# eloialonso/diamond

Measured on AMD Instinct MI355X. Metric: imagined frames/sec (64x64, 3 denoise steps, batch 256), higher is better.
Workload: dtype f32 via split-f16 MFMA (world-model convs (3x3 stride 1 / 2, 1x1): fp32 operands split into 2 x fp16 pieces, 3 x v_mfma_f32_*_f16 per product, fp32 accumulate (fp32-class, 22-bit operands); attention core, linears: exact fp32 v_mfma_f32_16x16x4_f32; actor-critic encoder forward, dgrad and weight-gra

## Files before the change

### diamond_amd/csrc/dmd_conv_f16ws.hip

```cpp
#include <type_traits>

#include "dmd_common.h"

typedef _Float16 h8 __attribute__((ext_vector_type(8)));
typedef _Float16 h4 __attribute__((ext_vector_type(4)));
typedef _Float16 h2 __attribute__((ext_vector_type(2)));
typedef float f32x16 __attribute__((ext_vector_type(16)));
typedef unsigned int u32x4 __attribute__((ext_vector_type(4)));

#ifdef DMD_LAB
#ifndef WS_ABL
#define WS_ABL 0
#endif
#else
#undef WS_ABL
#define WS_ABL 0
#endif
#if defined(DMD_LAB) && defined(WS_WRITEOUT_PRIO)
#define WS_PRIO_COMPUTE() __builtin_amdgcn_s_setprio(3)
#define WS_PRIO_WRITEOUT() __builtin_amdgcn_s_setprio(WS_WRITEOUT_PRIO)
#else
#define WS_PRIO_COMPUTE() do {} while (0)
#define WS_PRIO_WRITEOUT() do {} while (0)
#endif

template <bool B8_, int NCB_, int TAPS_ = 9>
struct WsGeom {
  static constexpr int NPT = 256;
  static constexpr bool B8 = B8_;
  static constexpr int NCB = NCB_;
  static constexpr int TAPS = TAPS_;
  static constexpr int COUT = 32 * NCB_;
  static constexpr int NPH = 4 / NCB_;
  static constexpr int SUB = B8_ ? 2 * NPH : NPH / 2;
  static constexpr int TS = B8_ ? 8 : 16;
  static constexpr int PW = TS + 2;
  static constexpr int PPS = PW * PW;
  static constexpr int NPP = SUB * PPS;
  static constexpr int ITEMS = (NPP * 4 + NPT - 1) / NPT;
  static constexpr int W_UNITS = TAPS_ * 2 * 2 * COUT;
  static constexpr int WU = (W_UNITS + 255) / 256;
  static constexpr int PATCH_BYTES = NPP * 64;
  static constexpr int W_BYTES = W_UNITS * 16;
  static constexpr int W_BASE = 2 * PATCH_BYTES;
  static constexpr int BUF_BYTES = PATCH_BYTES + W_BYTES;
  static constexpr int CIN_MAX = NCB_ == 2 ? 128 : 64;
  static constexpr int TAB_SLOTS = 4;
  static constexpr int TAB_FLOATS = TAB_SLOTS * SUB * CIN_MAX;
  static constexpr bool CD_TABLES = !(B8_ && NCB_ == 1);
  static constexpr int SMEM_BYTES = 2 * BUF_BYTES + (CD_TABLES ? 4 : 2) * TAB_FLOATS * 4 + COUT * 4;
  static constexpr bool DOUBLE_STAGE = NCB_ == 2;
  static constexpr bool ASM_LOADS = DOUBLE_STAGE;
  static constexpr int HALVES = TAPS_ * 2;
  static constexpr bool PL_REGS = !(B8_ && NCB_ == 1);
  static constexpr int blk_off(int blk) { return (B8_ ? (blk >> 1) * PPS + (blk & 1) * 4 * PW : blk * 2 * PW) * 64; }
  static constexpr bool PROJ = false;
  static constexpr int PROJ_KS = 1;
};

struct WsGeomProj : WsGeom<false, 2, 9> {
  static constexpr bool PROJ = true;
  static constexpr int PROJ_KS = 8;
  static constexpr int PROJ_BYTES = PROJ_KS * 2 * 2 * COUT * 16;
  static constexpr bool PL_REGS = false;
  static constexpr int SMEM_BYTES = WsGeom<false, 2, 9>::SMEM_BYTES + PROJ_BYTES;
};

struct WsTile {
  int n, y0, x0;
  bool valid;
};

template <class G>
__device__ __forceinline__ WsTile ws_subtile(const dmd_conv_params& p, int tile, int s) {
  const int tx = p.W / G::TS, per_img = tx * (p.H / G::TS);
  const int gs = tile * G::SUB + s;
  WsTile t;
  t.valid = gs < p.N * per_img;
  const int g2 = t.valid ? gs : 0;
  t.n = g2 / per_img;
  const int r = g2 - t.n * per_img;
  const int ty = r / tx;
  t.y0 = ty * G::TS;
  t.x0 = (r - ty * tx) * G::TS;
  return t;
}

__device__ __forceinline__ float ws_silu(float t) {
  return t * __builtin_amdgcn_rcpf(1.0f + __builtin_amdgcn_exp2f(-1.4426950408889634f * t));
}

template <int I, int N, class F>
__device__ __forceinline__ void ws_for(F&& f) {
  if constexpr (I < N) {
    f(std::integral_constant<int, I>{});
    ws_for<I + 1, N>(f);
  }
}

#ifndef WS_SYNCTHREADS
#define WS_SYNCTHREADS 0
#endif
__device__ __forceinline__ void ws_barrier() {
#if WS_SYNCTHREADS
  __syncthreads();
#else
  asm volatile("s_waitcnt lgkmcnt(0)\n\ts_barrier" ::: "memory");
#endif
}

#if defined(DMD_LAB) && defined(WS_TRACE)
#define WS_TRACE_WG (gridDim.x > 37 ? 37 : 0)
#define WS_TRACE_N 4096
__device__ unsigned long long ws_trace_buf[3][WS_TRACE_N];
__device__ int ws_trace_cnt[3];
#define WS_TRACE_DECL int ws_ti = 0
#define WS_STAMP(role_, tag_, step_)                                                                                  \
  do {                                                                                                                 \
    if (blockIdx.x == WS_TRACE_WG && (threadIdx.x & 255) == 0 && ws_ti < WS_TRACE_N) {                                  \
      ws_trace_buf[role_][ws_ti] = (__builtin_readcyclecounter() << 16) | ((unsigned long long)(tag_) << 12) | ((step_) & 0xfff); \
      ws_trace_cnt[role_] = ++ws_ti;                                                                                   \
    }                                                                                                                  \
  } while (0)
extern "C" int dmd_ws_trace_dump(unsigned long long* host, int* counts) {
  hipDeviceSynchronize();
  hipMemcpyFromSymbol(host, HIP_SYMBOL(ws_trace_buf), sizeof(unsigned long long) * 3 * WS_TRACE_N);
  hipMemcpyFromSymbol(counts, HIP_SYMBOL(ws_trace_cnt), sizeof(int) * 3);
  int zero[3] = {0, 0, 0};
  hipMemcpyToSymbol(HIP_SYMBOL(ws_trace_cnt), zero, sizeof(zero));
  return WS_TRACE_N;
}
#else
#define WS_TRACE_DECL
#define WS_STAMP(role_, tag_, step_) do {} while (0)
#endif

#ifndef WS_HOST_HELPERS
__device__ __forceinline__ void ws_aload(f32x4& dst, const f32x4* src) {
  asm volatile("global_load_dwordx4 %0, %1, off" : "=&v"(dst) : "v"(src) : "memory");
}
template <bool FIRST>
// ... 25 lines not shown
  const unsigned long long v = (unsigned long long)p;
  const unsigned lo = __builtin_amdgcn_readfirstlane((unsigned)v), hi = __builtin_amdgcn_readfirstlane((unsigned)(v >> 32));
  return (const char*)(((unsigned long long)hi << 32) | lo);
}
template <int CTRL, int ROW_MASK>
__device__ __forceinline__ double ws_dpp_add(double x) {
  const unsigned long long u = __builtin_bit_cast(unsigned long long, x);
  const unsigned lo = (unsigned)__builtin_amdgcn_update_dpp(0, (int)(unsigned)u, CTRL, ROW_MASK, 0xf, false);
  const unsigned hi = (unsigned)__builtin_amdgcn_update_dpp(0, (int)(unsigned)(u >> 32), CTRL, ROW_MASK, 0xf, false);
  return x + __builtin_bit_cast(double, (unsigned long long)lo | ((unsigned long long)hi << 32));
}
__device__ __forceinline__ double ws_wave_sum_lane63(double x) {
  x = ws_dpp_add<0xB1, 0xf>(x);
  x = ws_dpp_add<0x4E, 0xf>(x);
  x = ws_dpp_add<0x141, 0xf>(x);
  x = ws_dpp_add<0x140, 0xf>(x);
  x = ws_dpp_add<0x142, 0xa>(x);
  x = ws_dpp_add<0x143, 0xc>(x);
  return x;
}

#ifndef WS_HOST_HELPERS
template <int N, int M>
__device__ __forceinline__ void ws_await_set(f32x4 (&st)[M]) {
  static_assert(N >= 0 && N < 64, "vmcnt is a 6-bit field");
  static_assert(M == 6 || M == 7, "register sets of the double-staged geometries");
  if constexpr (M == 6)
    asm volatile("s_waitcnt vmcnt(%6) ; await %0 %1 %2 %3 %4 %5"
                 : "+v"(st[0]), "+v"(st[1]), "+v"(st[2]), "+v"(st[3]), "+v"(st[4]), "+v"(st[5]) : "n"(N) : "memory");
  else
    asm volatile("s_waitcnt vmcnt(%7) ; await %0 %1 %2 %3 %4 %5 %6"
                 : "+v"(st[0]), "+v"(st[1]), "+v"(st[2]), "+v"(st[3]), "+v"(st[4]), "+v"(st[5]), "+v"(st[6]) : "n"(N) : "memory");
}

template <int N, int M>
__device__ __forceinline__ void ws_use_all(f32x4 (&st)[M]) {
  static_assert(N <= M, "register set");
#pragma unroll
  for (int it = 0; it < N; ++it) asm volatile("; drained %0" : : "v"(st[it]));
}
#endif

struct WsA {
  h8 h, l;
};
struct WsB {
  h8 h0, h1, l0, l1;
};

struct WsAddr {
  int ph[3], pl[3];
  int w;
};

template <class G>
__device__ __forceinline__ void ws_addr_move(WsAddr& ad, int dpar) {
  const int dp = dpar * G::PATCH_BYTES, dw = dpar * G::W_BYTES;
#pragma unroll
  for (int dx = 0; dx < 3; ++dx) {
    ad.ph[dx] += dp;
    if (G::PL_REGS) ad.pl[dx] += dp;
  }
  ad.w += dw;
}

template <class G, int TAP>
struct WsWin {
  static constexpr int win = G::TAPS == 9 ? TAP : 4;
  static constexpr int dy = win / 3, dx = win % 3;
  static constexpr int off = (dy * G::PW + dx) * 64;
};

template <class G, int TAP, int BLK, bool LOW>
__device__ __forceinline__ h8 ws_read_b(const unsigned char* lds, const WsAddr& ad) {
  using Wn = WsWin<G, TAP>;
  return *(const h8*)(lds + (LOW ? (G::PL_REGS ? ad.pl[Wn::dx] : (ad.ph[Wn::dx] ^ 32)) : ad.ph[Wn::dx]) + (Wn::off + G::blk_off(BLK)));
}
template <class G, int TAP, bool LOW>
__device__ __forceinline__ h8 ws_read_a(const unsigned char* lds, const WsAddr& ad) {
  return *(const h8*)(lds + ad.w + (TAP * 2 + (LOW ? 1 : 0)) * 2 * G::COUT * 16);
}

template <class G, int P0, int NEXT, int NT, int NP0>
__device__ __forceinline__ void ws_halftap(f32x16 (&acc)[4], const WsA& a, const WsB& b, const unsigned char* lds, const WsAddr& ad,
                                           WsA& an, WsB& bn) {
#if WS_ABL & 16
  return;
#endif
  constexpr int P1 = P0 + 1, NP1 = NP0 + 1;
  acc[P0] = __builtin_amdgcn_mfma_f32_32x32x16_f16(a.h, b.h0, acc[P0], 0, 0, 0);
  if constexpr (NEXT == 3) an.h = ws_read_a<G, NT, false>(lds, ad);
  if constexpr (NEXT == 1 || NEXT == 2) bn.h0 = ws_read_b<G, NT, NP0, false>(lds, ad);
  __builtin_amdgcn_sched_barrier(0);
  acc[P1] = __builtin_amdgcn_mfma_f32_32x32x16_f16(a.h, b.h1, acc[P1], 0, 0, 0);
  if constexpr (NEXT == 3) bn.h0 = ws_read_b<G, NT, NP0, false>(lds, ad);
  if constexpr (NEXT == 1 || NEXT == 2) bn.h1 = ws_read_b<G, NT, NP1, false>(lds, ad);
  __builtin_amdgcn_sched_barrier(0);
  acc[P0] = __builtin_amdgcn_mfma_f32_32x32x16_f16(a.h, b.l0, acc[P0], 0, 0, 0);
  if constexpr (NEXT == 3) bn.h1 = ws_read_b<G, NT, NP1, false>(lds, ad);
  if constexpr (NEXT == 1 || NEXT == 2) bn.l0 = ws_read_b<G, NT, NP0, true>(lds, ad);
  __builtin_amdgcn_sched_barrier(0);
  acc[P1] = __builtin_amdgcn_mfma_f32_32x32x16_f16(a.h, b.l1, acc[P1], 0, 0, 0);
  if constexpr (NEXT == 3) bn.l0 = ws_read_b<G, NT, NP0, true>(lds, ad);
  if constexpr (NEXT == 1 || NEXT == 2) bn.l1 = ws_read_b<G, NT, NP1, true>(lds, ad);
  __builtin_amdgcn_sched_barrier(0);
  acc[P0] = __builtin_amdgcn_mfma_f32_32x32x16_f16(a.l, b.h0, acc[P0], 0, 0, 0);
  if constexpr (NEXT == 3) bn.l1 = ws_read_b<G, NT, NP1, true>(lds, ad);
  if constexpr (NEXT == 2) an.h = ws_read_a<G, NT + 1, false>(lds, ad);
  __builtin_amdgcn_sched_barrier(0);
  acc[P1] = __builtin_amdgcn_mfma_f32_32x32x16_f16(a.l, b.h1, acc[P1], 0, 0, 0);
  if constexpr (NEXT == 3) an.l = ws_read_a<G, NT, true>(lds, ad);
  if constexpr (NEXT == 2) an.l = ws_read_a<G, NT + 1, true>(lds, ad);
  __builtin_amdgcn_sched_barrier(0);
}

template <class G>
__device__ __forceinline__ void ws_chunk_body(f32x16 (&acc)[4], WsA& a, WsB& b, const unsigned char* lds, const WsAddr& ad) {
  WsA an = a;
  WsB bn = b;
  ws_for<0, G::HALVES - 1>([&](auto uc) {
    constexpr int U = decltype(uc)::value;
    constexpr int T = U / 2, H = U % 2;
    constexpr int NU = U + 1, NT = NU / 2, NH = NU % 2;
    constexpr int NEXT = (H == 0 && T + 1 < G::TAPS) ? 2 : 1;
    ws_halftap<G, 2 * H, NEXT, NT, 2 * NH>(acc, a, b, lds, ad, an, bn);
    b = bn;
    if (H == 1) a = an;
  });
}

template <class G>
__global__ __launch_bounds__(768, 3) void conv_f16ws_kernel(const dmd_conv_params p, int ntiles, int tiles_per_wg) {
  DMD_DYNAMIC_LDS(unsigned char, smem_raw);
  float* tab_a = (float*)(smem_raw + 2 * G::BUF_BYTES);
  float* tab_b = tab_a + G::TAB_FLOATS;
  float* tab_c = tab_b + G::TAB_FLOATS;
  float* tab_d = tab_c + G::TAB_FLOATS;
  float* bias_lds = tab_b + (G::CD_TABLES ? 3 : 1) * G::TAB_FLOATS;
  static_assert(G::SMEM_BYTES <= 160 * 1024, "LDS budget");
  unsigned char* proj_lds = (unsigned char*)(bias_lds + G::COUT);
  if constexpr (G::PROJ) {
    const u32x4* pwg = (const u32x4*)p.proj_w_f16;
    for (int u = (int)threadIdx.x; u < G::PROJ_BYTES / 16; u += 768) ((u32x4*)proj_lds)[u] = pwg[u];
  }

  const int role = __builtin_amdgcn_readfirstlane((int)(threadIdx.x >> 8));
  const int tid = (int)(threadIdx.x & 255);
  WS_TRACE_DECL;
  const int lane = tid & 63, wave = __builtin_amdgcn_readfirstlane(tid >> 6);
  WS_STAMP(role, 13, 0);
  const int up = p.upsample;
  const int Hs = p.H >> up, Ws = p.W >> up;
  const int Hv = p.valid_h ? p.valid_h : p.H, Wv = p.valid_w ? p.valid_w : p.W;
  const int Hvs = Hv >> up, Wvs = Wv >> up;
  const int C0 = p.src[0].C;
  const int C1 = p.nsrc > 1 ? p.src[1].C : 0;
  const int nch0 = C0 >> 4;
  const int nchunks = (C0 + C1) >> 4;
  const int tile0 = blockIdx.x * tiles_per_wg;
  const int nmy = min(tiles_per_wg, ntiles - tile0);
  const int S = nmy * nchunks;
  const int rot = (blockIdx.x * 7) % nmy;
#define WS_TILE(k) (tile0 + (((k) + rot) >= nmy ? (k) + rot - nmy : (k) + rot))

  if (role == 2) {
    const int q = tid & 3;
    constexpr bool IPOS_REGS = !(G::B8 && G::NCB == 1);
    auto ipos_calc = [&](int it, int t) -> int {
      const int pp = (it * G::NPT + t) >> 2;
      const bool ok = pp < G::NPP;
      const int s = G::SUB == 1 ? 0 : (ok ? pp / G::PPS : 0);
      const int rem = pp - s * G::PPS;
      const int py = rem / G::PW, px = rem - py * G::PW;
      return ok ? ((s << 16) | (py << 8) | px) : -1;
    };
    int ipos_[IPOS_REGS ? G::ITEMS : 1];
#pragma unroll
    for (int it = 0; it < (IPOS_REGS ? G::ITEMS : 1); ++it) ipos_[it] = ipos_calc(it, tid);
    auto ipos = [&](int it) -> int {
      if (IPOS_REGS) return ipos_[IPOS_REGS ? it : 0];
      int t = tid;
      WS_OPAQUE(t);
      return ipos_calc(it, t);
    };
    auto loff_of = [&](int it) {
      int t = tid;
      if (G::SUB > 1) WS_OPAQUE(t);
      const int qq = t & 3;
      return ((it * (G::NPT / 4) + (t >> 2)) * 4 + (((qq >> 1) + ((ipos(it) & 0xff) >> 1)) & 3)) * 2 + (qq & 1);
    };
    int gk = -1;
    int tab_n[G::SUB];
#pragma unroll
    for (int s2 = 0; s2 < G::SUB; ++s2) tab_n[s2] = -1;
    int tab_slot = -1;
    WsTile ti[G::SUB];
    int goff[G::ITEMS];
    unsigned gzero = 0;
    int gtile = 0;
    auto item_source = [&](int it, bool& inb) -> int {
      const int ip = ipos(it);
      const int s = ip >> 16, py = (ip >> 8) & 0xff, px = ip & 0xff;
      const WsTile t = G::SUB == 1 ? ti[0] : ws_subtile<G>(p, gtile, s);
      const int iy = t.y0 - 1 + py, ix = t.x0 - 1 + px;
      const bool window = G::TAPS == 9 || (py >= 1 && py <= G::TS && px >= 1 && px <= G::TS);
      inb = ip >= 0 && window && t.valid && iy >= 0 && iy < Hv && ix >= 0 && ix < Wv;
      return inb ? ((t.n * Hs + (iy >> up)) * Ws + (ix >> up)) : 0;
    };

    auto setup_tile = [&](int k) {
// ... 162 lines not shown
          }
#else
#pragma unroll
          for (int el = 0; el < 4; ++el) {
            const float y = t[i][el] * u[i][el];
            u[i][el] = zero ? 0.f : y;
          }
#endif
        }
        __builtin_amdgcn_sched_barrier(0);
#endif
#pragma unroll
        for (int i = 0; i < NB; ++i) {
          const int it = I0 + i;
          const float* x = u[i];
          const unsigned h01 = __builtin_bit_cast(unsigned, (h2){(_Float16)x[0], (_Float16)x[1]});
          const unsigned h23 = __builtin_bit_cast(unsigned, (h2){(_Float16)x[2], (_Float16)x[3]});
          const unsigned l01 = ws_low_pair(x[0], x[1], h01);
          const unsigned l23 = ws_low_pair(x[2], x[3], h23);
          if ((it + 1) * G::NPT <= G::NPP * 4 || ipos(it) >= 0) {
            const int lo = loff_of(it);
            pb[lo] = (uint2){h01, h23};
            pb[lo ^ 4] = (uint2){l01, l23};
          }
        }
        __builtin_amdgcn_sched_barrier(0);
      });
      if constexpr (BATCH != G::ITEMS) reissue();
    };

    f32x4 stage0[G::ITEMS], stage1[G::DOUBLE_STAGE ? G::ITEMS : 1];
    unsigned zm0 = 0, zm1 = 0;
    int sl0 = 0, sl1 = 0;
    if constexpr (G::DOUBLE_STAGE) {
      issue_S(0, stage0, zm0, sl0);
      issue_S(1, stage1, zm1, sl1);
      WS_STAMP(2, 14, 0);
      ws_barrier();
      WS_STAMP(2, 15, 0);
      stage_S(0, stage0, zm0, sl0, 2);
      WS_STAMP(2, 12, 0);
      ws_barrier();
      for (int j = 0; j < S; j += 2) {
        WS_STAMP(2, 0, j);
        if (j + 1 < S) {
          stage_S(j + 1, stage1, zm1, sl1, j + 3);
          WS_STAMP(2, 1, j);
          WS_STAMP(2, 2, j);
        }
        ws_barrier();
        WS_STAMP(2, 3, j);
        if (j + 1 < S) {
          WS_STAMP(2, 0, j + 1);
          if (j + 2 < S) {
            stage_S(j + 2, stage0, zm0, sl0, j + 4);
            WS_STAMP(2, 1, j + 1);
            WS_STAMP(2, 2, j + 1);
          }
          ws_barrier();
          WS_STAMP(2, 3, j + 1);
        }
      }
      if constexpr (G::ASM_LOADS) {
        WS_WAIT_VM(0);
        ws_use_all<G::ITEMS>(stage0);
        ws_use_all<G::ITEMS>(stage1);
      }
    } else {
      issue_S(0, stage0, zm0, sl0);
      ws_barrier();
      stage_S(0, stage0, zm0, sl0, S > 1 ? 1 : -1);
      ws_barrier();
      for (int j = 0; j < S; ++j) {
        WS_STAMP(2, 0, j);
        if (j + 1 < S) {
          stage_S(j + 1, stage0, zm0, sl0, j + 2 < S ? j + 2 : -1);
          WS_STAMP(2, 1, j);
          WS_STAMP(2, 2, j);
        }
        ws_barrier();
        WS_STAMP(2, 3, j);
      }
    }
  } else {
    __builtin_amdgcn_s_setprio(3);
    const int cb = wave % G::NCB;
    const int ph = wave / G::NCB;
    const int n31 = lane & 31, g = lane >> 5;
    WsAddr ad;
    {
      const int col = G::B8 ? (n31 & 7) : (n31 & 15);
      const int pixbase = G::B8 ? (ph * 2 * G::PPS + (n31 >> 3) * G::PW + col)
                                : ((ph >> 1) * G::PPS + ((ph & 1) * 8 + (n31 >> 4)) * G::PW + col);
#pragma unroll
      for (int dx = 0; dx < 3; ++dx) {
        ad.ph[dx] = (pixbase * 4 + ((g + ((col + dx) >> 1)) & 3)) * 16;
        ad.pl[dx] = ad.ph[dx] ^ 32;
      }
      ad.w = G::W_BASE + (g * G::COUT + cb * 32 + n31) * 16;
    }
    int apar = 0;
    const unsigned char* lds = smem_raw;

    f32x16 acc[4];

    constexpr int NPO = G::B8 ? 2 : 1;
    int pixoff_[NPO];
    auto pixoff_of = [&](int blk) {
      const int base = pixoff_[G::B8 ? (blk >> 1) : 0];
      const int rows = G::B8 ? (blk & 1) * 4 : blk * 2;
      return base < 0 ? -1 : base + rows * p.W * (G::COUT / 4);
    };
    int dead = 0;
    constexpr int NSTAT = G::B8 ? 2 : 1;
    int stat_slot[NSTAT];
    using StatAcc = std::conditional_t<G::B8 || G::PROJ, float, double>;
    StatAcc ssum[NSTAT], ssq[NSTAT];
    int pending = 4;
    constexpr bool RES_PREFETCH = G::NCB == 2 && !G::PROJ;
    f32x4 rnext[4];
    auto res_prefetch = [&](int blk) __attribute__((always_inline)) {
      const int po = pixoff_of(blk);
#pragma unroll
      for (int qd = 0; qd < 4; ++qd)
        rnext[qd] = (p.residual && po >= 0 && !(WS_ABL & 128)) ? *(const f32x4*)(p.residual + (size_t)po * 4 + 8 * qd) : (f32x4){0.f, 0.f, 0.f, 0.f};
    };
    f32x4 xq[G::PROJ ? 2 * G::PROJ_KS : 1];
    auto proj_fetch_unit = [&](int blk, auto uc) __attribute__((always_inline)) {
      if constexpr (G::PROJ) {
        constexpr int u = decltype(uc)::value;
        const int po = pixoff_of(blk);
        const unsigned boff = po < 0 ? 0u : ((((unsigned)(po - (cb * 8 + g)) >> 4) << 8) + 32u * g);
        const char* xs = (const char*)p.proj_x[u / 4] + boff + (u % 4) * 64;
        xq[2 * u] = *(const f32x4*)xs;
        xq[2 * u + 1] = *(const f32x4*)(xs + 16);
      }
    };
    auto proj_mfma_unit = [&](f32x16& dacc, auto uc) __attribute__((always_inline)) {
      if constexpr (G::PROJ) {
        constexpr int ks = decltype(uc)::value;
        const unsigned char* pw = proj_lds + (ad.w - G::W_BASE - apar * G::W_BYTES);
        const f32x4 x0 = xq[2 * ks], x1 = xq[2 * ks + 1];
        const unsigned h01 = __builtin_bit_cast(unsigned, (h2){(_Float16)x0[0], (_Float16)x0[1]});
        const unsigned h23 = __builtin_bit_cast(unsigned, (h2){(_Float16)x0[2], (_Float16)x0[3]});
        const unsigned h45 = __builtin_bit_cast(unsigned, (h2){(_Float16)x1[0], (_Float16)x1[1]});
        const unsigned h67 = __builtin_bit_cast(unsigned, (h2){(_Float16)x1[2], (_Float16)x1[3]});
        const h8 xh = __builtin_bit_cast(h8, (u32x4){h01, h23, h45, h67});
        const h8 xl = __builtin_bit_cast(h8, (u32x4){ws_low_pair(x0[0], x0[1], h01), ws_low_pair(x0[2], x0[3], h23),
                                                     ws_low_pair(x1[0], x1[1], h45), ws_low_pair(x1[2], x1[3], h67)});
        const h8 wh = *(const h8*)(pw + (ks * 2 + 0) * 2 * G::COUT * 16);
        const h8 wl = *(const h8*)(pw + (ks * 2 + 1) * 2 * G::COUT * 16);
        dacc = __builtin_amdgcn_mfma_f32_32x32x16_f16(wh, xh, dacc, 0, 0, 0);
        dacc = __builtin_amdgcn_mfma_f32_32x32x16_f16(wh, xl, dacc, 0, 0, 0);
        dacc = __builtin_amdgcn_mfma_f32_32x32x16_f16(wl, xh, dacc, 0, 0, 0);
      }
    };
    auto epi_begin = [&](int k) {
      const int tile = WS_TILE(k);
#pragma unroll
      for (int s = 0; s < NPO; ++s) {
        const WsTile t = ws_subtile<G>(p, tile, G::B8 ? ph * 2 + s : (ph >> 1));
        int oy, ox;
        int n31e = n31;
        if constexpr (G::PROJ) {
          int te = tid;
          WS_OPAQUE(te);
          n31e = te & 31;
        }
        if (G::B8) {
          oy = t.y0 + (n31e >> 3);
          ox = t.x0 + (n31e & 7);
        } else {
          oy = t.y0 + (ph & 1) * 8 + (n31e >> 4);
          ox = t.x0 + (n31e & 15);
        }
        pixoff_[s] = t.valid ? (((t.n * p.H + oy) * p.W + ox) * (G::COUT / 4) + cb * 8 + g) : -1;
        if constexpr (!G::PROJ) {
          if (s == 0) dead = 0;
#pragma unroll
          for (int b = 0; b < (G::B8 ? 2 : 4); ++b) {
            const int blk = G::B8 ? 2 * s + b : b;
            const int row = oy + (G::B8 ? b * 4 : b * 2);
            dead |= (row >= Hv || ox >= Wv) ? (1 << blk) : 0;
          }
        }
      }
#pragma unroll
      for (int kk = 0; kk < NSTAT; ++kk) {
        const WsTile t = ws_subtile<G>(p, tile, G::B8 ? ph * 2 + kk : (ph >> 1));
        int T, tt;
        if (G::B8) {
          const int tx8 = p.W / 8;
          T = tx8 * (p.H / 8);
          tt = (t.y0 / 8) * tx8 + t.x0 / 8;
        } else {
          const int tx16 = p.W / 16;
          T = tx16 * (p.H / 8);
          tt = (t.y0 / 8 + (ph & 1)) * tx16 + t.x0 / 16;
        }
        stat_slot[kk] = t.valid ? ((t.n * G::NCB + cb) * T + tt) : -1;
        ssum[kk] = 0;
        ssq[kk] = 0;
      }
      pending = 0;
      if (RES_PREFETCH) res_prefetch(0);
    };
    auto epi_blocks = [&](int count, bool land = false) {
      const int first = pending, last = min(4, pending + count);
#pragma unroll
      for (int blk = 0; blk < 4; ++blk) {
        if (blk < first || blk >= last) continue;
        if (G::NCB == 1 && p.out_nchw) {
          if (pixoff_of(blk) >= 0 && g == 0) {
            const int pixel = pixoff_of(blk) >> 3;
            const int HW = p.H * p.W;
            const int n = pixel / HW, rem = pixel - n * HW;
#pragma unroll
            for (int c = 0; c < 4; ++c)
              if (c < p.Cout) p.out[((size_t)n * p.Cout + c) * HW + rem] = acc[blk][c];
          }
          continue;
        }
        const int po = pixoff_of(blk);
        if (po >= 0) {
          float* op = p.out + (size_t)po * 4;
          if (!RES_PREFETCH && !G::PROJ) res_prefetch(blk);
          if constexpr (G::PROJ) {
            ws_for<0, 4>([&](auto bc) {
              if (decltype(bc)::value == blk) {
                ws_for<0, G::PROJ_KS>([&](auto uc) { proj_fetch_unit(blk, uc); });
                ws_for<0, G::PROJ_KS>([&](auto uc) {
                  proj_mfma_unit(acc[blk], uc);
                  __builtin_amdgcn_sched_barrier(0);
                });
              }
            });
          }
          f32x4 v[4];
#pragma unroll
          for (int qd = 0; qd < 4; ++qd) {
            v[qd] = (f32x4){acc[blk][4 * qd], acc[blk][4 * qd + 1], acc[blk][4 * qd + 2], acc[blk][4 * qd + 3]};
            if (!G::PROJ) {
#pragma unroll
              for (int r = 0; r < 4; ++r) v[qd][r] += rnext[qd][r];
            }
          }
          if (land) {
            WS_WAIT_VM(0);
            land = false;
          }
          float fs = 0.f, fq = 0.f;
#pragma unroll
          for (int qd = 0; qd < 4; ++qd) {
            if (!(WS_ABL & 128) || v[qd][0] == 1.2345e30f) *(f32x4*)(op + 8 * qd) = v[qd];
            fs += (v[qd][0] + v[qd][1]) + (v[qd][2] + v[qd][3]);
            fq = __builtin_fmaf(v[qd][0], v[qd][0], fq);
            fq = __builtin_fmaf(v[qd][1], v[qd][1], fq);
            fq = __builtin_fmaf(v[qd][2], v[qd][2], fq);
            fq = __builtin_fmaf(v[qd][3], v[qd][3], fq);
          }
          if (!G::PROJ && ((dead >> blk) & 1)) {
            fs = 0.f;
            fq = 0.f;
          }
          if (RES_PREFETCH && blk + 1 < 4) res_prefetch(blk + 1);
          const int slot = G::B8 ? (blk >> 1) : 0;
          ssum[slot] += (StatAcc)fs;
          ssq[slot] += (StatAcc)fq;
        }
      }
      if (land) WS_WAIT_VM(0);
      pending = last;
      if (last == 4 && first < 4 && p.out_stats) {
#pragma unroll
        for (int kk = 0; kk < NSTAT; ++kk) {
          const double a = ws_wave_sum_lane63((double)ssum[kk]);
          const double b = ws_wave_sum_lane63((double)ssq[kk]);
          if (lane == 63 && stat_slot[kk] >= 0) {
            double* o = p.out_stats + (size_t)stat_slot[kk] * 2;
            o[0] = a;
            o[1] = b;
          }
        }
      }
    };
    auto proj_step = [&](auto sc, bool wnext) __attribute__((always_inline)) {
      if constexpr (G::PROJ) {
        constexpr int blk = decltype(sc)::value;
        const int po = pixoff_of(blk);
        ws_for<0, G::PROJ_KS>([&](auto uc) {
          proj_mfma_unit(acc[blk], uc);
          if constexpr (blk + 1 < 4) proj_fetch_unit(blk + 1, uc);
          __builtin_amdgcn_sched_barrier(0);
        });
        if (wnext) {
          if constexpr (blk + 1 < 4)
            WS_WAIT_VM(16);
          else
            WS_WAIT_VM(0);
        }
        if (po >= 0) {
          float* op = p.out + (size_t)po * 4;
          float fs = 0.f, fq = 0.f;
#pragma unroll
          for (int qd = 0; qd < 4; ++qd) {
            const f32x4 v = (f32x4){acc[blk][4 * qd], acc[blk][4 * qd + 1], acc[blk][4 * qd + 2], acc[blk][4 * qd + 3]};
            if (!(WS_ABL & 128) || v[0] == 1.2345e30f) *(f32x4*)(op + 8 * qd) = v;
            fs += (v[0] + v[1]) + (v[2] + v[3]);
            fq = __builtin_fmaf(v[0], v[0], fq);
            fq = __builtin_fmaf(v[1], v[1], fq);
            fq = __builtin_fmaf(v[2], v[2], fq);
            fq = __builtin_fmaf(v[3], v[3], fq);
          }
          ssum[0] += (StatAcc)fs;
          ssq[0] += (StatAcc)fq;
        }
        pending = blk + 1;
        if constexpr (blk == 3) {
          if (p.out_stats) {
            const double a = ws_wave_sum_lane63((double)ssum[0]);
            const double b = ws_wave_sum_lane63((double)ssq[0]);
            if (lane == 63 && stat_slot[0] >= 0) {
              double* o = p.out_stats + (size_t)stat_slot[0] * 2;
              o[0] = a;
              o[1] = b;
            }
          }
        }
      }
    };
    const int blocks_per_step = nchunks >= 4 ? 1 : (nchunks >= 2 ? 2 : 4);

    const u32x4* cwglob = (const u32x4*)p.w_f16;
    auto cons_load_W = [&](int ck, int wbuf) {
#if WS_ABL & 32
      if (wbuf >= 0) return;
#endif
      const u32x4* w = cwglob + (size_t)ck * G::W_UNITS + tid;
      u32x4* wl = (u32x4*)(smem_raw + G::W_BASE + wbuf * G::W_BYTES) + wave * 64;
#pragma unroll
      for (int i = 0; i < G::WU; ++i)
        if (G::W_UNITS % 256 == 0 || 256 * i + wave * 64 < G::W_UNITS)
          __builtin_amdgcn_global_load_lds((const __attribute__((address_space(1))) void*)(w + 256 * i),
                                           (__attribute__((address_space(3))) void*)(wl + 256 * i), 16, 0, 0);
    };
    auto cons_land_W = [&]() { WS_WAIT_VM(0); };

    if (role == 0 && tid < G::COUT)
      bias_lds[tid] = (p.bias ? p.bias[tid] : 0.f) + ((G::PROJ && p.proj_bias) ? p.proj_bias[tid] : 0.f);
    WS_STAMP(role, 14, 0);
    ws_barrier();
    WS_STAMP(role, 15, 0);
    if (role == 1) {
      cons_load_W(0, 0);
      cons_land_W();
    }
    WS_STAMP(role, 12, 0);
    ws_barrier();
    int j = 0;
    int k = role;
    if (role == 1 && nmy > 0) {
      for (int ck = 0; ck < nchunks; ++ck, ++j) {
        const bool wnext = j + 1 < S;
        WS_STAMP(role, 8, j);
        if (wnext) {
          cons_load_W((j + 1) % nchunks, (j + 1) & 1);
          cons_land_W();
        }
        WS_STAMP(role, 10, j);
        ws_barrier();
        WS_STAMP(role, 11, j);
      }
    }
    for (; k < nmy; k += 2) {
      if (!G::PROJ && pending < 4) epi_blocks(4);
      WS_PRIO_COMPUTE();
      {
        f32x4 bq[4];
#pragma unroll
        for (int qd = 0; qd < 4; ++qd) bq[qd] = *(const f32x4*)(bias_lds + cb * 32 + 8 * qd + 4 * g);
#pragma unroll
        for (int blk = 0; blk < 4; ++blk)
#pragma unroll
          for (int r = 0; r < 16; ++r) acc[blk][r] = bq[r >> 2][r & 3];
      }
      ws_addr_move<G>(ad, (j & 1) - apar);
      apar = j & 1;
      WsA a, an;
      WsB b, bn;
      a.h = ws_read_a<G, 0, false>(lds, ad);
      b.h0 = ws_read_b<G, 0, 0, false>(lds, ad);
      b.h1 = ws_read_b<G, 0, 1, false>(lds, ad);
      b.l0 = ws_read_b<G, 0, 0, true>(lds, ad);
      b.l1 = ws_read_b<G, 0, 1, true>(lds, ad);
      a.l = ws_read_a<G, 0, true>(lds, ad);
      an = a;
      bn = b;
      constexpr int LH = (G::HALVES - 1) % 2;
      for (int ck = 0; ck < nchunks; ++ck, ++j) {
        WS_STAMP(role, 4, j);
        ws_chunk_body<G>(acc, a, b, lds, ad);
        WS_STAMP(role, 5, j);
        ws_barrier();
        WS_STAMP(role, 6, j);
        ws_addr_move<G>(ad, 1 - 2 * apar);
        apar ^= 1;
        ws_halftap<G, 2 * LH, 3, 0, 0>(acc, a, b, lds, ad, an, bn);
        a = an;
        b = bn;
      }
      epi_begin(k);
      if (k + 1 >= nmy) break;
      WS_PRIO_WRITEOUT();
      if constexpr (G::PROJ) {
        ws_for<0, 4>([&](auto sc) {
          const bool wnext = j + 1 < S;
          WS_STAMP(role, 8, j);
          if constexpr (decltype(sc)::value == 0) ws_for<0, G::PROJ_KS>([&](auto uc) { proj_fetch_unit(0, uc); });
          if (wnext) cons_load_W((j + 1) % nchunks, (j + 1) & 1);
          WS_STAMP(role, 9, j);
          proj_step(sc, wnext);
          WS_STAMP(role, 10, j);
          ws_barrier();
          WS_STAMP(role, 11, j);
          ++j;
        });
      } else {
        for (int ck = 0; ck < nchunks; ++ck, ++j) {
          const bool wnext = j + 1 < S;
          WS_STAMP(role, 8, j);
          if (wnext) cons_load_W((j + 1) % nchunks, (j + 1) & 1);
          WS_STAMP(role, 9, j);
          if (pending < 4)
            epi_blocks(blocks_per_step, wnext);
          else if (wnext)
            cons_land_W();
          WS_STAMP(role, 10, j);
          ws_barrier();
          WS_STAMP(role, 11, j);
        }
      }
    }
    WS_STAMP(role, 13, 1);
    if (pending < 4) epi_blocks(4);
    WS_STAMP(role, 13, 2);
  }
#undef WS_TILE
}

template <class G>
static int launch_f16ws(const dmd_conv_params& p, int ntiles, hipStream_t st) {
  static bool attr_set[DMD_MAX_DEVICES] = {};
  static int ncus[DMD_MAX_DEVICES] = {};
  int dev = 0;
  if (hipGetDevice(&dev) != hipSuccess || dev < 0 || dev >= DMD_MAX_DEVICES) dev = 0;
  if (!attr_set[dev]) {
    hipError_t e = hipFuncSetAttribute(reinterpret_cast<const void*>(&conv_f16ws_kernel<G>), hipFuncAttributeMaxDynamicSharedMemorySize,
                                       G::SMEM_BYTES);
    DMD_CHECK_ARG(e == hipSuccess, "conv_f16ws: hipFuncSetAttribute(%d bytes): %s", G::SMEM_BYTES, hipGetErrorString(e));
    int n = 0;
    if (hipDeviceGetAttribute(&n, hipDeviceAttributeMultiprocessorCount, dev) != hipSuccess || n <= 0) n = 256;
    ncus[dev] = n;
    attr_set[dev] = true;
  }
  const int ncu = ncus[dev];
  const int tpw = (ntiles + ncu - 1) / ncu;
  const int nwg = (ntiles + tpw - 1) / tpw;
  hipLaunchKernelGGL((conv_f16ws_kernel<G>), dim3(nwg), dim3(768), G::SMEM_BYTES, st, p, ntiles, tpw);
  return 0;
}

extern "C" int dmd_conv2d_proj_eligible(const dmd_conv_params* p);
int dmd_launch_conv_f16ws(const dmd_conv_params& p, hipStream_t st) {
  const bool b8 = p.W % 16 != 0;
  const int sub8 = p.N * (p.H / 8) * (p.W / 8), t16 = p.N * (p.H / 16) * (p.W / 16);
  if (p.proj_nsrc) {
    DMD_CHECK_ARG(dmd_conv2d_proj_eligible(&p), "conv: the fused skip projection needs a split-fp16 3x3 stride-1 launch with Cout 64, "
                  "H, W multiples of 16, two 64-channel projection sources and no other residual (dmd_conv2d_proj_eligible)");
    return launch_f16ws<WsGeomProj>(p, t16, st);
  }
  if (p.taps == 9) {
    if (p.CoutPad == 64) return b8 ? launch_f16ws<WsGeom<true, 2, 9>>(p, (sub8 + 3) / 4, st) : launch_f16ws<WsGeom<false, 2, 9>>(p, t16, st);
    return b8 ? launch_f16ws<WsGeom<true, 1, 9>>(p, (sub8 + 7) / 8, st) : launch_f16ws<WsGeom<false, 1, 9>>(p, (t16 + 1) / 2, st);
  }
  if (p.CoutPad == 64) return b8 ? launch_f16ws<WsGeom<true, 2, 1>>(p, (sub8 + 3) / 4, st) : launch_f16ws<WsGeom<false, 2, 1>>(p, t16, st);
  return b8 ? launch_f16ws<WsGeom<true, 1, 1>>(p, (sub8 + 7) / 8, st) : launch_f16ws<WsGeom<false, 1, 1>>(p, (t16 + 1) / 2, st);
}

__global__ void pack_weight_f16x2_kernel(const float* __restrict__ oihw, _Float16* __restrict__ packed, int Cout, int Cin,
                                         int CinPad, int taps) {
  const size_t total = (size_t)(CinPad / 16) * taps * Cout * 16;
  const size_t idx = (size_t)blockIdx.x * blockDim.x + threadIdx.x;
  if (idx >= total) return;
  const int e = idx % 8;
  const int co = (idx / 8) % Cout;
  const int g = (idx / (8 * (size_t)Cout)) % 2;
  const int tap = (idx / (8 * (size_t)Cout * 2)) % taps;
  const int chunk = idx / (8 * (size_t)Cout * 2 * taps);
  const int c = chunk * 16 + g * 8 + e;
  float v = 0.f;
  if (c < Cin) v = oihw[((size_t)co * Cin + c) * taps + tap];
  const _Float16 h = (_Float16)v;
  const _Float16 l = (_Float16)(v - (float)h);
  const size_t base = ((((size_t)chunk * taps + tap) * 2 + 0) * 2 + g) * ((size_t)Cout * 8) + (size_t)co * 8 + e;
  packed[base] = h;
  packed[base + 2 * (size_t)Cout * 8] = l;
}

extern "C" int dmd_pack_conv_weight_f16x2(const float* oihw, void* packed, int Cout, int Cin, int k, int CinPad,
                                          dmd_stream_t stream) {
  DMD_CHECK_ARG(oihw && packed, "pack_f16x2: null");
  DMD_CHECK_ARG((Cout == 64 || Cout == 32) && (k == 3 || k == 1) && CinPad >= Cin && CinPad % 16 == 0,
                "pack_f16x2: needs Cout in {32, 64} (got %d), k in {1, 3}, CinPad %% 16 == 0", Cout);
  const int taps = k * k;
  const size_t total = (size_t)(CinPad / 16) * taps * Cout * 16;
  hipLaunchKernelGGL(pack_weight_f16x2_kernel, dim3((unsigned)((total + 255) / 256)), dim3(256), 0, (hipStream_t)stream, oihw,
                     (_Float16*)packed, Cout, Cin, CinPad, taps);
  DMD_LAUNCH_CHECK();
  return 0;
}

extern "C" int dmd_conv2d_f16x2_eligible(const dmd_conv_params* p) {
  if (!p || (p->precision & 0xff) != DMD_PRECISION_F16X2 || !p->w_f16) return 0;
  if (p->stride != 1 || p->residual_norm.stats || (p->taps != 9 && p->taps != 1)) return 0;
  if (p->taps == 1 && p->upsample) return 0;
  for (int i = 0; i < p->nsrc; ++i)
    if (p->src[i].prologue != DMD_PROLOGUE_NONE && p->src[i].C % DMD_GN_GROUP != 0) return 0;
  const bool head = p->out_nchw && p->Cout <= 4 && p->CoutPad == 32 && !p->residual && !p->out_stats;
  if (!head && ((p->Cout != 64 && p->Cout != 32) || p->CoutPad != p->Cout || p->out_nchw)) return 0;
  int cin = 0;
  for (int i = 0; i < p->nsrc; ++i) cin += p->src[i].C;
  if (cin > (p->CoutPad == 64 ? 128 : 64)) return 0;
  const long long src_pixels = (long long)p->N * (p->H >> p->upsample) * (p->W >> p->upsample);
  if (src_pixels >= (1ll << 24)) return 0;
  for (int i = 0; i < p->nsrc; ++i)
    if (src_pixels * p->src[i].C * 4 >= (1ll << 32)) return 0;
  const bool a16 = p->H % 16 == 0 && p->W % 16 == 0;
  const bool b8 = p->W % 16 != 0;
  return (a16 || b8) ? 1 : 0;
}

extern "C" int dmd_conv2d_proj_eligible(const dmd_conv_params* p) {
  if (!p || !dmd_conv2d_f16x2_eligible(p)) return 0;
  if (p->taps != 9 || p->upsample || p->Cout != 64 || p->CoutPad != 64 || p->out_nchw || p->residual) return 0;
  if (p->H % 16 != 0 || p->W % 16 != 0 || p->valid_h || p->valid_w) return 0;
  if (p->nsrc != 1 || p->src[0].C != 64) return 0;
  if ((long long)p->N * p->H * p->W * 256 >= (1ll << 32)) return 0;
  if (p->proj_nsrc != 2 || !p->proj_w_f16 || !p->proj_x[0] || !p->proj_x[1] || p->proj_C[0] != 64 || p->proj_C[1] != 64) return 0;
  return 1;
}
```

Before: 12640.

## Use two-block waves for 32-cout 16x16 3x3 convs to double tile count

Adds a geometry variant in which each consumer wave computes two 32x32 output blocks instead of four for the 32-channel, 16x16, 3x3 conv path. Each workgroup then covers one 16x16 subtile instead of two, doubling the tile count so more workgroups can fill the CUs. Per-tile statistics are now combined across wave pairs through a small LDS slot, which adds extra barriers. The old wide layout stays available behind an environment variable, and a launch-plan query hook is added.

```diff
diff --git a/diamond_amd/csrc/dmd_conv_f16ws.hip b/diamond_amd/csrc/dmd_conv_f16ws.hip
--- a/diamond_amd/csrc/dmd_conv_f16ws.hip
+++ b/diamond_amd/csrc/dmd_conv_f16ws.hip
@@ -24,15 +24,18 @@
 #define WS_PRIO_WRITEOUT() do {} while (0)
 #endif
 
-template <bool B8_, int NCB_, int TAPS_ = 9>
-struct WsGeom {
+template <bool B8_, int NCB_, int TAPS_, int NBLK_>
+struct WsGeomBase {
+  static_assert(NBLK_ == 4 || (NBLK_ == 2 && !B8_ && NCB_ == 1), "two-block waves: 16x16 patches x 32 couts only");
   static constexpr int NPT = 256;
   static constexpr bool B8 = B8_;
   static constexpr int NCB = NCB_;
   static constexpr int TAPS = TAPS_;
+  static constexpr int NBLK = NBLK_;
   static constexpr int COUT = 32 * NCB_;
   static constexpr int NPH = 4 / NCB_;
-  static constexpr int SUB = B8_ ? 2 * NPH : NPH / 2;
+  static constexpr int SUB = B8_ ? 2 * NPH : NPH * NBLK_ / 8;
+  static constexpr bool STAT_PAIR = NBLK_ == 2;
   static constexpr int TS = B8_ ? 8 : 16;
   static constexpr int PW = TS + 2;
   static constexpr int PPS = PW * PW;
@@ -48,15 +51,19 @@
   static constexpr int TAB_SLOTS = 4;
   static constexpr int TAB_FLOATS = TAB_SLOTS * SUB * CIN_MAX;
   static constexpr bool CD_TABLES = !(B8_ && NCB_ == 1);
-  static constexpr int SMEM_BYTES = 2 * BUF_BYTES + (CD_TABLES ? 4 : 2) * TAB_FLOATS * 4 + COUT * 4;
-  static constexpr bool DOUBLE_STAGE = NCB_ == 2;
+  static constexpr int PAIR_BYTES = STAT_PAIR ? 2 * 2 * 64 * 16 : 0;
+  static constexpr int SMEM_BYTES = 2 * BUF_BYTES + (CD_TABLES ? 4 : 2) * TAB_FLOATS * 4 + COUT * 4 + PAIR_BYTES;
+  static constexpr bool DOUBLE_STAGE = NCB_ == 2 || NBLK_ == 2;
   static constexpr bool ASM_LOADS = DOUBLE_STAGE;
-  static constexpr int HALVES = TAPS_ * 2;
+  static constexpr int HALVES = TAPS_ * NBLK_ / 2;
   static constexpr bool PL_REGS = !(B8_ && NCB_ == 1);
   static constexpr int blk_off(int blk) { return (B8_ ? (blk >> 1) * PPS + (blk & 1) * 4 * PW : blk * 2 * PW) * 64; }
   static constexpr bool PROJ = false;
   static constexpr int PROJ_KS = 1;
 };
+template <bool B8_, int NCB_, int TAPS_ = 9>
+struct WsGeom : WsGeomBase<B8_, NCB_, TAPS_, (!B8_ && NCB_ == 1 && TAPS_ == 9) ? 2 : 4> {};
+struct WsGeomC32Wide : WsGeomBase<false, 1, 9, 4> {};
 
 struct WsGeomProj : WsGeom<false, 2, 9> {
   static constexpr bool PROJ = true;
@@ -248,7 +255,7 @@
 }
 
 template <class G, int P0, int NEXT, int NT, int NP0>
-__device__ __forceinline__ void ws_halftap(f32x16 (&acc)[4], const WsA& a, const WsB& b, const unsigned char* lds, const WsAddr& ad,
+__device__ __forceinline__ void ws_halftap(f32x16 (&acc)[G::NBLK], const WsA& a, const WsB& b, const unsigned char* lds, const WsAddr& ad,
                                            WsA& an, WsB& bn) {
 #if WS_ABL & 16
   return;
@@ -256,42 +263,45 @@
   constexpr int P1 = P0 + 1, NP1 = NP0 + 1;
   acc[P0] = __builtin_amdgcn_mfma_f32_32x32x16_f16(a.h, b.h0, acc[P0], 0, 0, 0);
   if constexpr (NEXT == 3) an.h = ws_read_a<G, NT, false>(lds, ad);
-  if constexpr (NEXT == 1 || NEXT == 2) bn.h0 = ws_read_b<G, NT, NP0, false>(lds, ad);
+  if constexpr (NEXT == 1 || NEXT == 2 || NEXT == 4) bn.h0 = ws_read_b<G, NT, NP0, false>(lds, ad);
   __builtin_amdgcn_sched_barrier(0);
   acc[P1] = __builtin_amdgcn_mfma_f32_32x32x16_f16(a.h, b.h1, acc[P1], 0, 0, 0);
   if constexpr (NEXT == 3) bn.h0 = ws_read_b<G, NT, NP0, false>(lds, ad);
-  if constexpr (NEXT == 1 || NEXT == 2) bn.h1 = ws_read_b<G, NT, NP1, false>(lds, ad);
+  if constexpr (NEXT == 1 || NEXT == 2 || NEXT == 4) bn.h1 = ws_read_b<G, NT, NP1, false>(lds, ad);
   __builtin_amdgcn_sched_barrier(0);
   acc[P0] = __builtin_amdgcn_mfma_f32_32x32x16_f16(a.h, b.l0, acc[P0], 0, 0, 0);
   if constexpr (NEXT == 3) bn.h1 = ws_read_b<G, NT, NP1, false>(lds, ad);
-  if constexpr (NEXT == 1 || NEXT == 2) bn.l0 = ws_read_b<G, NT, NP0, true>(lds, ad);
+  if constexpr (NEXT == 1 || NEXT == 2 || NEXT == 4) bn.l0 = ws_read_b<G, NT, NP0, true>(lds, ad);
   __builtin_amdgcn_sched_barrier(0);
   acc[P1] = __builtin_amdgcn_mfma_f32_32x32x16_f16(a.h, b.l1, acc[P1], 0, 0, 0);
   if constexpr (NEXT == 3) bn.l0 = ws_read_b<G, NT, NP0, true>(lds, ad);
-  if constexpr (NEXT == 1 || NEXT == 2) bn.l1 = ws_read_b<G, NT, NP1, true>(lds, ad);
+  if constexpr (NEXT == 1 || NEXT == 2 || NEXT == 4) bn.l1 = ws_read_b<G, NT, NP1, true>(lds, ad);
   __builtin_amdgcn_sched_barrier(0);
   acc[P0] = __builtin_amdgcn_mfma_f32_32x32x16_f16(a.l, b.h0, acc[P0], 0, 0, 0);
   if constexpr (NEXT == 3) bn.l1 = ws_read_b<G, NT, NP1, true>(lds, ad);
   if constexpr (NEXT == 2) an.h = ws_read_a<G, NT + 1, false>(lds, ad);
+  if constexpr (NEXT == 4) an.h = ws_read_a<G, NT, false>(lds, ad);
   __builtin_amdgcn_sched_barrier(0);
   acc[P1] = __builtin_amdgcn_mfma_f32_32x32x16_f16(a.l, b.h1, acc[P1], 0, 0, 0);
   if constexpr (NEXT == 3) an.l = ws_read_a<G, NT, true>(lds, ad);
   if constexpr (NEXT == 2) an.l = ws_read_a<G, NT + 1, true>(lds, ad);
+  if constexpr (NEXT == 4) an.l = ws_read_a<G, NT, true>(lds, ad);
   __builtin_amdgcn_sched_barrier(0);
 }
 
 template <class G>
-__device__ __forceinline__ void ws_chunk_body(f32x16 (&acc)[4], WsA& a, WsB& b, const unsigned char* lds, const WsAddr& ad) {
+__device__ __forceinline__ void ws_chunk_body(f32x16 (&acc)[G::NBLK], WsA& a, WsB& b, const unsigned char* lds, const WsAddr& ad) {
   WsA an = a;
   WsB bn = b;
+  constexpr int HPT = G::NBLK / 2;
   ws_for<0, G::HALVES - 1>([&](auto uc) {
     constexpr int U = decltype(uc)::value;
-    constexpr int T = U / 2, H = U % 2;
-    constexpr int NU = U + 1, NT = NU / 2, NH = NU % 2;
-    constexpr int NEXT = (H == 0 && T + 1 < G::TAPS) ? 2 : 1;
+    constexpr int T = U / HPT, H = U % HPT;
+    constexpr int NU = U + 1, NT = NU / HPT, NH = NU % HPT;
+    constexpr int NEXT = HPT == 1 ? 4 : ((H == 0 && T + 1 < G::TAPS) ? 2 : 1);
     ws_halftap<G, 2 * H, NEXT, NT, 2 * NH>(acc, a, b, lds, ad, an, bn);
     b = bn;
-    if (H == 1) a = an;
+    if (H == HPT - 1) a = an;
   });
 }
 
@@ -620,16 +630,18 @@
         WS_STAMP(2, 3, j);
       }
     }
+    if constexpr (G::STAT_PAIR) ws_barrier();
   } else {
     __builtin_amdgcn_s_setprio(3);
     const int cb = wave % G::NCB;
     const int ph = wave / G::NCB;
+    const int wave_sub = (ph * 2 * G::NBLK) >> 4, wave_row = (ph * 2 * G::NBLK) & 15;
     const int n31 = lane & 31, g = lane >> 5;
     WsAddr ad;
     {
       const int col = G::B8 ? (n31 & 7) : (n31 & 15);
       const int pixbase = G::B8 ? (ph * 2 * G::PPS + (n31 >> 3) * G::PW + col)
-                                : ((ph >> 1) * G::PPS + ((ph & 1) * 8 + (n31 >> 4)) * G::PW + col);
+                                : (wave_sub * G::PPS + (wave_row + (n31 >> 4)) * G::PW + col);
 #pragma unroll
       for (int dx = 0; dx < 3; ++dx) {
         ad.ph[dx] = (pixbase * 4 + ((g + ((col + dx) >> 1)) & 3)) * 16;
@@ -640,7 +652,7 @@
     int apar = 0;
     const unsigned char* lds = smem_raw;
 
-    f32x16 acc[4];
+    f32x16 acc[G::NBLK];
 
     constexpr int NPO = G::B8 ? 2 : 1;
     int pixoff_[NPO];
@@ -654,8 +666,11 @@
     int stat_slot[NSTAT];
     using StatAcc = std::conditional_t<G::B8 || G::PROJ, float, double>;
     StatAcc ssum[NSTAT], ssq[NSTAT];
-    int pending = 4;
-    constexpr bool RES_PREFETCH = G::NCB == 2 && !G::PROJ;
+    float fsk[G::STAT_PAIR ? 2 : 1], fqk[G::STAT_PAIR ? 2 : 1];
+    bool stat_fin = false;
+    double* pair_slot = (double*)(bias_lds + G::COUT) + ((role * 2 + (wave >> 1)) * 64 + lane) * 2;
+    int pending = G::NBLK;
+    constexpr bool RES_PREFETCH = (G::NCB == 2 || G::NBLK == 2) && !G::PROJ;
     f32x4 rnext[4];
     auto res_prefetch = [&](int blk) __attribute__((always_inline)) {
       const int po = pixoff_of(blk);
@@ -697,7 +712,7 @@
       const int tile = WS_TILE(k);
 #pragma unroll
       for (int s = 0; s < NPO; ++s) {
-        const WsTile t = ws_subtile<G>(p, tile, G::B8 ? ph * 2 + s : (ph >> 1));
+        const WsTile t = ws_subtile<G>(p, tile, G::B8 ? ph * 2 + s : wave_sub);
         int oy, ox;
         int n31e = n31;
         if constexpr (G::PROJ) {
@@ -709,14 +724,14 @@
           oy = t.y0 + (n31e >> 3);
           ox = t.x0 + (n31e & 7);
         } else {
-          oy = t.y0 + (ph & 1) * 8 + (n31e >> 4);
+          oy = t.y0 + wave_row + (n31e >> 4);
           ox = t.x0 + (n31e & 15);
         }
         pixoff_[s] = t.valid ? (((t.n * p.H + oy) * p.W + ox) * (G::COUT / 4) + cb * 8 + g) : -1;
         if constexpr (!G::PROJ) {
           if (s == 0) dead = 0;
 #pragma unroll
-          for (int b = 0; b < (G::B8 ? 2 : 4); ++b) {
+          for (int b = 0; b < (G::B8 ? 2 : G::NBLK); ++b) {
             const int blk = G::B8 ? 2 * s + b : b;
             const int row = oy + (G::B8 ? b * 4 : b * 2);
             dead |= (row >= Hv || ox >= Wv) ? (1 << blk) : 0;
@@ -725,7 +740,7 @@
       }
 #pragma unroll
       for (int kk = 0; kk < NSTAT; ++kk) {
-        const WsTile t = ws_subtile<G>(p, tile, G::B8 ? ph * 2 + kk : (ph >> 1));
+        const WsTile t = ws_subtile<G>(p, tile, G::B8 ? ph * 2 + kk : wave_sub);
         int T, tt;
         if (G::B8) {
           const int tx8 = p.W / 8;
@@ -734,19 +749,20 @@
         } else {
           const int tx16 = p.W / 16;
           T = tx16 * (p.H / 8);
-          tt = (t.y0 / 8 + (ph & 1)) * tx16 + t.x0 / 16;
+          tt = (t.y0 / 8 + (wave_row >> 3)) * tx16 + t.x0 / 16;
         }
         stat_slot[kk] = t.valid ? ((t.n * G::NCB + cb) * T + tt) : -1;
         ssum[kk] = 0;
         ssq[kk] = 0;
       }
+      if constexpr (G::STAT_PAIR) fsk[0] = fsk[1] = fqk[0] = fqk[1] = 0.f;
       pending = 0;
       if (RES_PREFETCH) res_prefetch(0);
     };
     auto epi_blocks = [&](int count, bool land = false) {
-      const int first = pending, last = min(4, pending + count);
-#pragma unroll
-      for (int blk = 0; blk < 4; ++blk) {
+      const int first = pending, last = min(G::NBLK, pending + count);
+#pragma unroll
+      for (int blk = 0; blk < G::NBLK; ++blk) {
         if (blk < first || blk >= last) continue;
         if (G::NCB == 1 && p.out_nchw) {
           if (pixoff_of(blk) >= 0 && g == 0) {
@@ -801,15 +817,29 @@
             fs = 0.f;
             fq = 0.f;
           }
-          if (RES_PREFETCH && blk + 1 < 4) res_prefetch(blk + 1);
-          const int slot = G::B8 ? (blk >> 1) : 0;
-          ssum[slot] += (StatAcc)fs;
-          ssq[slot] += (StatAcc)fq;
+          if (RES_PREFETCH && blk + 1 < G::NBLK) res_prefetch(blk + 1);
+          if constexpr (G::STAT_PAIR) {
+            fsk[blk] = fs;
+            fqk[blk] = fq;
+          } else {
+            const int slot = G::B8 ? (blk >> 1) : 0;
+            ssum[slot] += (StatAcc)fs;
+            ssq[slot] += (StatAcc)fq;
+          }
         }
       }
       if (land) WS_WAIT_VM(0);
       pending = last;
-      if (last == 4 && first < 4 && p.out_stats) {
+      if constexpr (G::STAT_PAIR) {
+        if (last == G::NBLK && first < G::NBLK && p.out_stats) {
+          if (wave & 1) {
+            stat_fin = true;
+          } else {
+            pair_slot[0] = (0.0 + (double)fsk[0]) + (double)fsk[1];
+            pair_slot[1] = (0.0 + (double)fqk[0]) + (double)fqk[1];
+          }
+        }
+      } else if (last == G::NBLK && first < G::NBLK && p.out_stats) {
 #pragma unroll
         for (int kk = 0; kk < NSTAT; ++kk) {
           const double a = ws_wave_sum_lane63((double)ssum[kk]);
@@ -867,7 +897,26 @@
         }
       }
     };
-    const int blocks_per_step = nchunks >= 4 ? 1 : (nchunks >= 2 ? 2 : 4);
+    auto stat_finish = [&]() {
+      if constexpr (G::STAT_PAIR) {
+        if (stat_fin) {
+          stat_fin = false;
+          double s = pair_slot[0], q = pair_slot[1];
+          s += (double)fsk[0];
+          q += (double)fqk[0];
+          s += (double)fsk[1];
+          q += (double)fqk[1];
+          const double a = ws_wave_sum_lane63(s);
+          const double b = ws_wave_sum_lane63(q);
+          if (lane == 63 && stat_slot[0] >= 0) {
+            double* o = p.out_stats + (size_t)stat_slot[0] * 2;
+            o[0] = a;
+            o[1] = b;
+          }
+        }
+      }
+    };
+    const int blocks_per_step = nchunks >= G::NBLK ? 1 : (2 * nchunks >= G::NBLK ? 2 : 4);
 
     const u32x4* cwglob = (const u32x4*)p.w_f16;
     auto cons_load_W = [&](int ck, int wbuf) {
@@ -911,14 +960,15 @@
       }
     }
     for (; k < nmy; k += 2) {
-      if (!G::PROJ && pending < 4) epi_blocks(4);
+      if (!G::PROJ && !G::STAT_PAIR && pending < G::NBLK) epi_blocks(G::NBLK);
+      stat_finish();
       WS_PRIO_COMPUTE();
       {
         f32x4 bq[4];
 #pragma unroll
         for (int qd = 0; qd < 4; ++qd) bq[qd] = *(const f32x4*)(bias_lds + cb * 32 + 8 * qd + 4 * g);
 #pragma unroll
-        for (int blk = 0; blk < 4; ++blk)
+        for (int blk = 0; blk < G::NBLK; ++blk)
 #pragma unroll
           for (int r = 0; r < 16; ++r) acc[blk][r] = bq[r >> 2][r & 3];
       }
@@ -934,7 +984,7 @@
       a.l = ws_read_a<G, 0, true>(lds, ad);
       an = a;
       bn = b;
-      constexpr int LH = (G::HALVES - 1) % 2;
+      constexpr int LH = (G::HALVES - 1) % (G::NBLK / 2);
       for (int ck = 0; ck < nchunks; ++ck, ++j) {
         WS_STAMP(role, 4, j);
         ws_chunk_body<G>(acc, a, b, lds, ad);
@@ -969,10 +1019,12 @@
           WS_STAMP(role, 8, j);
           if (wnext) cons_load_W((j + 1) % nchunks, (j + 1) & 1);
           WS_STAMP(role, 9, j);
-          if (pending < 4)
+          if (pending < G::NBLK) {
             epi_blocks(blocks_per_step, wnext);
-          else if (wnext)
-            cons_land_W();
+          } else {
+            stat_finish();
+            if (wnext) cons_land_W();
+          }
           WS_STAMP(role, 10, j);
           ws_barrier();
           WS_STAMP(role, 11, j);
@@ -980,10 +1032,22 @@
       }
     }
     WS_STAMP(role, 13, 1);
-    if (pending < 4) epi_blocks(4);
+    if (pending < G::NBLK) epi_blocks(G::NBLK);
+    if constexpr (G::STAT_PAIR) {
+      ws_barrier();
+      stat_finish();
+    }
     WS_STAMP(role, 13, 2);
   }
 #undef WS_TILE
+}
+
+static std::atomic<long long> ws_last_plan{0};
+extern "C" void dmd_conv_f16ws_last_launch(int* tiles, int* tiles_per_wg, int* workgroups) {
+  const long long v = ws_last_plan.load(std::memory_order_relaxed);
+  *tiles = (int)(v >> 40);
+  *tiles_per_wg = (int)((v >> 20) & 0xfffff);
+  *workgroups = (int)(v & 0xfffff);
 }
 
 template <class G>
@@ -1004,9 +1068,12 @@
   const int ncu = ncus[dev];
   const int tpw = (ntiles + ncu - 1) / ncu;
   const int nwg = (ntiles + tpw - 1) / tpw;
+  ws_last_plan.store(((long long)ntiles << 40) | ((long long)(tpw & 0xfffff) << 20) | (nwg & 0xfffff), std::memory_order_relaxed);
   hipLaunchKernelGGL((conv_f16ws_kernel<G>), dim3(nwg), dim3(768), G::SMEM_BYTES, st, p, ntiles, tpw);
   return 0;
 }
+
+static DmdEnvInt c32_tile{"DIAMOND_C32_TILE", 256};
 
 extern "C" int dmd_conv2d_proj_eligible(const dmd_conv_params* p);
 int dmd_launch_conv_f16ws(const dmd_conv_params& p, hipStream_t st) {
@@ -1019,7 +1086,10 @@
   }
   if (p.taps == 9) {
     if (p.CoutPad == 64) return b8 ? launch_f16ws<WsGeom<true, 2, 9>>(p, (sub8 + 3) / 4, st) : launch_f16ws<WsGeom<false, 2, 9>>(p, t16, st);
-    return b8 ? launch_f16ws<WsGeom<true, 1, 9>>(p, (sub8 + 7) / 8, st) : launch_f16ws<WsGeom<false, 1, 9>>(p, (t16 + 1) / 2, st);
+    if (b8) return launch_f16ws<WsGeom<true, 1, 9>>(p, (sub8 + 7) / 8, st);
+    const int tile = c32_tile.get();
+    DMD_CHECK_ARG(tile == 256 || tile == 512, "conv: DIAMOND_C32_TILE is 256 or 512 (got %d)", tile);
+    return tile == 512 ? launch_f16ws<WsGeomC32Wide>(p, (t16 + 1) / 2, st) : launch_f16ws<WsGeom<false, 1, 9>>(p, t16, st);
   }
   if (p.CoutPad == 64) return b8 ? launch_f16ws<WsGeom<true, 2, 1>>(p, (sub8 + 3) / 4, st) : launch_f16ws<WsGeom<false, 2, 1>>(p, t16, st);
   return b8 ? launch_f16ws<WsGeom<true, 1, 1>>(p, (sub8 + 7) / 8, st) : launch_f16ws<WsGeom<false, 1, 1>>(p, (t16 + 1) / 2, st);
```

Result: faster. 12890, median of 6 (+2.0%).
